# MCV-Univalle/HM-OpenCL

Measured on AMD Instinct MI355X. Metric: GSAD/s, higher is better.
Workload: dtype u8

## Files before the change

### hm-opencl_amd/csrc/hmme.hip

```cpp
#include "../../include/hmme.h"
#include "../../include/hmme_test.h"

#include <hip/hip_runtime.h>

#include <climits>
#include <cmath>
#include <cstdarg>
#include <cstdio>
#include <cstdlib>
#include <cstring>
#include <functional>
#include <string>
#include <type_traits>
#include <vector>

#include "me_kernels.hpp"

using hmme::MeJob;
using hmme::MeJob16;
using hmme::RefSet;

namespace {
constexpr int kMarginX = 128;
constexpr int kMarginY = 80;
// ... 1194 lines not shown
    if (t < best * 0.999) { best = t; best_k = k; }
  }
  return best_k;
}

static int plan_tail8(int tail, int slots, int w, int tail_knob) {
  if (tail <= 0 || tail >= hmme::kSegPrepThreads) return 0;
  const int nt = hmme::me_num_tasks(w, w), units = (nt + hmme::kSegUnit - 1) / hmme::kSegUnit;
  const long total = (long)tail * units;
  int best_wgs = 0;
  double best = (double)units + 0.25;
  for (int rounds = 1; rounds <= 4; ++rounds) {
    const long wgs = std::max<long>(1, std::min<long>((long)rounds * slots, total));
    const double per_wg = (double)total / wgs;
    const double t = 1.08 * rounds * (std::ceil(per_wg) + 0.25 * (1.0 + (per_wg - 1.0) / units)) + 0.5;
    if (t < best * 0.999) { best = t; best_wgs = (int)wgs; }
    if (wgs < (long)rounds * slots) break;
  }
  if (tail_knob > 1) best_wgs = (int)std::max<long>(1, std::min<long>((long)tail * tail_knob, total));
  return best_wgs;
}
static bool tail_one_launch(int head, int n_tail, int launches_knob) { return launches_knob == 1 || (launches_knob != 2 && 3 * n_tail >= head); }

static FramePlan plan_search(int jobs, int n_refs, int slots, int search_range, bool wide, const Knobs& knobs) {
  FramePlan pl;
  const int w = 2 * search_range + 1, tail = jobs % slots;
  pl.jobs = pl.tail_first = jobs;
  if (wide) {
    pl.mode = SearchMode::kStrips16;
    pl.pdw = pick_pdw16(w);
    const int rmax = pl.strip_rows = rows_max16(pl.pdw), n_min = strips_for(pl.pdw, w);
    const int h = hmme::me_strip_rows16(w, w, rmax, n_min + 4);
    pl.n_strips = (w + h - 1) / h;
    const int lanes = (((w + 1) >> 1) + 2) / 3;
    auto strip_cost = [&](int k) {
      const int hk = (w + k - 1) / k;
      return 2.0 * ((((hk * lanes + 63) >> 6) + 3) >> 2) + 1.0;
    };
    if (tail && knobs.tail_parts != 1) {
      const int k_max = std::min(w / 4, 64);
      int k = knobs.tail_parts > 1 ? std::min(knobs.tail_parts, k_max) : plan_tail(tail, slots, pl.n_strips, k_max, strip_cost);
      if (k < pl.n_strips) k = pl.n_strips;
      if (k > pl.n_strips) { pl.tail_first = jobs - tail; pl.tail_parts = k; }
    }
    pl.n_wg16 = pl.tail_first * pl.n_strips + (jobs - pl.tail_first) * pl.tail_parts;
    pl.table_bytes = sizeof(MeJob16) * (size_t)pl.n_wg16;
  } else if (search_range > 64) {
    pl.mode = SearchMode::kTiles8;
    pl.table_bytes = sizeof(MeJob16) * (size_t)jobs * 4;
  } else {
    const int wgs = tail && knobs.tail_parts != 1 ? plan_tail8(tail, slots, w, knobs.tail_parts) : 0;
    if (wgs > 0) { pl.tail_first = jobs - tail; pl.tail_wgs = wgs; }
    const int head = pl.tail_first, n_tail = jobs - head;
    if (!n_tail) {
      pl.table_bytes = sizeof(MeJob) * (size_t)head;
    } else if (tail_one_launch(head, n_tail, knobs.tail_launches)) {
      pl.mode = SearchMode::kSegments8;
      pl.table_bytes = hmme::me_seg_table_bytes(head + wgs, jobs);
    } else {
      pl.mode = SearchMode::kHeadThenSegments8;
      pl.tail_jobs_off = (sizeof(MeJob) * (size_t)head + 255) & ~(size_t)255;
      pl.table_bytes = pl.tail_jobs_off + hmme::me_seg_table_bytes(wgs, n_tail);
    }
  }
  pl.first_strip = pl.mode != SearchMode::kWhole8;
  const size_t per_ref = n_refs > 0 ? (pl.table_bytes + n_refs - 1) / n_refs : pl.table_bytes;
  pl.table_grow = per_ref * hmme::kMaxRefs + 4096;
  return pl;
}
static FramePlan plan_launch(const hmme_ctx* ctx, const hmme_frame_params* fp, int count, int n_refs, bool force16 = false) {
  return plan_search(count * n_refs, n_refs, ctx->wg_slots, fp->search_range, fp->bit_depth > 8 || force16, knobs());
}

int hmme_test_tail_plan(int width, int height, int search_range, int n_pairs, int slots, int* out) {
  if (!out || width < 8 || height < 8 || width > 16384 || height > 16384 || search_range < 1 || search_range > 64 || n_pairs < 1 || slots < 1) return HMME_ERR_ARG;
  const FramePlan pl = plan_search(hmme_num_ctus(width, height) * n_pairs, n_pairs, slots, search_range, false, Knobs{});
  out[0] = pl.jobs; out[1] = pl.tail_first; out[2] = pl.tail_wgs; out[3] = pl.mode == SearchMode::kSegments8 ? 1 : 0;
  return HMME_OK;
}

int hmme_test_pk_gate(uint32_t lambda_q16) { return hmme::me_pk_gate(lambda_q16) ? 1 : 0; }
int hmme_test_pk_body(uint32_t lambda_q16, int fen) { return hmme::me_pk_body(lambda_q16, fen ? 1 : 0); }
int hmme_test_pk_task_marker_free(int wx, int wy, int k, int it0, int n_it) { return hmme::me_task_marker_free(wx, wy, k, it0, n_it) ? 1 : 0; }

static int prep_jobs(hmme_ctx* ctx, const hmme_plane* cur, const hmme_frame_params* fp, const void* d_pred_q, int first, int count,
                     int n_refs, hipStream_t s, const FramePlan& pl, const void* d_center_q = nullptr) {
  const int jobs = pl.jobs, head = pl.tail_first, n_tail = jobs - head, w = cur->width, h = cur->height, sr = fp->search_range;
  bool moved;
  int rc = ensure(ctx, ctx->buf[kJobs], pl.table_bytes, pl.table_grow, &moved);
  if (moved) ctx->jobs_tag.valid = false;
  if (rc) return rc;
  if (pl.first_strip) {
    rc = ensure(ctx, ctx->buf[kFirstStrip], sizeof(int) * (size_t)jobs, sizeof(int) * (size_t)(jobs / (n_refs > 0 ? n_refs : 1) + 1) * hmme::kMaxRefs, &moved);
    if (moved) ctx->jobs_tag.valid = false;
    if (rc) return rc;
  }
  void* const d_jobs = ctx->buf[kJobs].p;
  int* const d_first_strip = ctx->buf[kFirstStrip].as<int>();
  hmme_ctx::TableTag tag;
  tag.valid = !d_pred_q && !d_center_q;
  tag.w = w; tag.h = h; tag.sr = sr; tag.first = first; tag.count = count; tag.pairs = n_refs;
  tag.bit_depth = fp->bit_depth | (pl.mode == SearchMode::kStrips16 && fp->bit_depth == 8 ? 0x100 : 0);
  tag.buf = d_jobs; tag.buf2 = pl.first_strip ? d_first_strip : nullptr; tag.stream = (void*)s;
  if (tag.same(ctx->jobs_tag)) return HMME_OK;
  ctx->jobs_tag.valid = false;
  const dim3 block(256);
  const auto grid = [](int n) { return dim3((n + 255) / 256); };
  const int16_t* pred = (const int16_t*)d_pred_q;
  switch (pl.mode) {
    case SearchMode::kTiles8:
      hipLaunchKernelGGL(hmme::me_prep_jobs_tile_kernel, grid(jobs), block, 0, s, (MeJob16*)d_jobs, d_first_strip, pred, first, count, n_refs, w, h, sr);
      break;
    case SearchMode::kStrips16:
      hipLaunchKernelGGL(hmme::me_prep_jobs16_kernel, grid(jobs), block, 0, s, (MeJob16*)d_jobs, d_first_strip, pred, first, count, n_refs, w, h, sr,
                         pl.n_strips, pl.strip_rows, pl.tail_first, pl.tail_parts, (const int16_t*)d_center_q);
      break;
    case SearchMode::kWhole8:
    case SearchMode::kSegments8:
    case SearchMode::kHeadThenSegments8: {
      const int idx0 = pl.mode == SearchMode::kSegments8 ? head : 0;
      if (head && idx0)
        hipLaunchKernelGGL(hmme::me_prep_whole_segments_kernel, grid(head), block, 0, s, d_jobs, d_first_strip, pred, first, count, n_refs, w, h, sr,
                           head + pl.tail_wgs, head);
      else if (head)
        hipLaunchKernelGGL(hmme::me_prep_jobs_kernel, grid(head), block, 0, s, (MeJob*)d_jobs, pred, first, count, n_refs, w, h, sr, 0, head, 1,
                           (uint32_t*)nullptr, (const int16_t*)nullptr);
      if (n_tail)
        hipLaunchKernelGGL(hmme::me_prep_segments_kernel, dim3(1), dim3(hmme::kSegPrepThreads), 0, s, (void*)((uint8_t*)d_jobs + pl.tail_jobs_off), d_first_strip,
                           pred, first, count, n_refs, w, h, sr, idx0 + pl.tail_wgs, head, n_tail, idx0);
      break;
    }
  }
  HIP_TRY(ctx, hipGetLastError());
  ctx->jobs_tag = tag;
  return HMME_OK;
}

static int run_search(hmme_ctx* ctx, const RefSet& curs, int cur_ctus_x, const RefSet& refs, int ref_pitch, const hmme_frame_params* fp, const FramePlan& pl,
                      int16_t* d_mv, uint32_t* d_sad, hipStream_t s) {
  const int head = pl.tail_first, n_tail = pl.jobs - head;
  const bool one_launch = pl.mode == SearchMode::kSegments8;
  const void* const d_jobs = ctx->buf[kJobs].p;
  const int* const d_first_strip = ctx->buf[kFirstStrip].as<int>();
  switch (pl.mode) {
    case SearchMode::kStrips16:
      return launch_search16(ctx, curs, cur_ctus_x, refs, ref_pitch, (const MeJob16*)d_jobs, d_first_strip, pl.jobs, pl.n_wg16,
                             pl.pdw, pl.strip_rows, fp->fen, fp->bit_depth, d_mv, d_sad, s);
    case SearchMode::kTiles8:
      return launch_search8_split(ctx, curs, cur_ctus_x, refs, ref_pitch, (const MeJob16*)d_jobs, d_first_strip, pl.jobs, 4,
                                  fp->fen, d_mv, d_sad, s);
    case SearchMode::kWhole8:
      return launch_search8<0>(ctx, curs, cur_ctus_x, refs, ref_pitch, d_jobs, head, fp->fen, d_mv, d_sad, nullptr, 0, s);
    case SearchMode::kSegments8:
    case SearchMode::kHeadThenSegments8: break;
  }
  unsigned long long* best = nullptr;
  int rc = merge_table(ctx, one_launch ? pl.jobs : n_tail, nullptr, s, &best);
  if (rc) return rc;
  if (one_launch)
    return launch_search8_segments(ctx, curs, cur_ctus_x, refs, ref_pitch, d_jobs, d_first_strip, pl.jobs, head + pl.tail_wgs, fp->fen, d_mv, d_sad, s, best);
  rc = launch_search8<0>(ctx, curs, cur_ctus_x, refs, ref_pitch, d_jobs, head, fp->fen, d_mv, d_sad, nullptr, 0, s);
  if (rc) return rc;
  return launch_search8_segments(ctx, curs, cur_ctus_x, refs, ref_pitch, (const uint8_t*)d_jobs + pl.tail_jobs_off, d_first_strip, n_tail, pl.tail_wgs,
                                 fp->fen, d_mv + (size_t)head * 2 * HMME_NUM_CTU_PARTS, d_sad + (size_t)head * HMME_NUM_CTU_PARTS, s, best);
}

// ... 2426 lines not shown
```

### hm-opencl_amd/csrc/me_kernels.hpp

```cpp
#pragma once

#include <hip/hip_runtime.h>
#include <stdint.h>

namespace hmme {

constexpr int kParts = 593;
constexpr int kPDW = 49;
constexpr int kWinRowsMax = 192;
constexpr int kIdxBits = 10;
constexpr uint32_t kInvCost = 3146751u;
constexpr int kGroups = 10;
constexpr int kIterPerTask = 4;
constexpr int kIterPerTaskSplit = 1;
static_assert(kIterPerTask == 4 && kIterPerTaskSplit <= 4, "2 iteration bits in the key; the guided schedule deals 4 / 2 / 1");
constexpr int kThreads = 256;

struct MeJob {
  int16_t ctu_x, ctu_y;
  int16_t lt_x, lt_y;
  int16_t rb_x, rb_y;
  int16_t pred_x, pred_y;
};
static_assert(sizeof(MeJob) == 16, "MeJob layout");
constexpr int kMaxRefs = 16;
struct RefSet { const uint8_t* base[kMaxRefs]; };

#include "me_slotmap.inc"

typedef uint16_t u16x4_t __attribute__((ext_vector_type(4)));
typedef uint32_t u32x2_t __attribute__((ext_vector_type(2)));
typedef __attribute__((address_space(3))) char lds_char_t;
typedef volatile __attribute__((address_space(3))) uint64_t lds_vu64_t;
typedef volatile __attribute__((address_space(3), aligned(4))) uint64_t lds_vu64a4_t;

__device__ __forceinline__ uint64_t me_pkadd(uint64_t a, uint64_t b) { return a + b; }
__device__ __forceinline__ uint64_t me_pksub(uint64_t a, uint64_t b) {
  return ((uint64_t)((uint32_t)(a >> 32) - (uint32_t)(b >> 32)) << 32) | (uint64_t)((uint32_t)a - (uint32_t)b);
}

#define ME_MAXKEY 0xFFFFFFFFu
#define ME_QSAD(pair, cur, acc) __builtin_amdgcn_qsad_pk_u16_u8((pair), (cur), (acc))
#define ME_KEYS(v, p, mult)                                                                                    \
  uint32_t v##_0, v##_1, v##_2, v##_3;                                                                         \
  asm volatile("v_mad_u32_u16 %0, %1, %2, %3" : "=v"(v##_0) : "v"((uint32_t)(p)), "s"(mult), "v"(c0));                   \
  asm volatile("v_mad_u32_u16 %0, %1, %2, %3 op_sel:[1,0,0,0]" : "=v"(v##_1) : "v"((uint32_t)(p)), "s"(mult), "v"(c1));   \
  asm volatile("v_mad_u32_u16 %0, %1, %2, %3" : "=v"(v##_2) : "v"((uint32_t)((p) >> 32)), "s"(mult), "v"(c2));           \
  asm volatile("v_mad_u32_u16 %0, %1, %2, %3 op_sel:[1,0,0,0]" : "=v"(v##_3) : "v"((uint32_t)((p) >> 32)), "s"(mult), "v"(c3))
#define ME_LIN(v, a, b)                                                                                         \
  uint32_t v##_0, v##_1, v##_2, v##_3;                                                                          \
  asm volatile("v_add3_u32 %0, %1, %2, %3" : "=v"(v##_0) : "v"(a##_0), "v"(b##_0), "v"(nc0));                              \
  asm volatile("v_add3_u32 %0, %1, %2, %3" : "=v"(v##_1) : "v"(a##_1), "v"(b##_1), "v"(nc1));                              \
  asm volatile("v_add3_u32 %0, %1, %2, %3" : "=v"(v##_2) : "v"(a##_2), "v"(b##_2), "v"(nc2));                              \
  asm volatile("v_add3_u32 %0, %1, %2, %3" : "=v"(v##_3) : "v"(a##_3), "v"(b##_3), "v"(nc3))
#define ME_SUB(v, a, b)                                                                                         \
  uint32_t v##_0, v##_1, v##_2, v##_3;                                                                          \
  asm volatile("v_sad_u32 %0, %1, %2, %3" : "=v"(v##_0) : "v"(a##_0), "v"(b##_0), "v"(c0));                                \
  asm volatile("v_sad_u32 %0, %1, %2, %3" : "=v"(v##_1) : "v"(a##_1), "v"(b##_1), "v"(c1));                                \
  asm volatile("v_sad_u32 %0, %1, %2, %3" : "=v"(v##_2) : "v"(a##_2), "v"(b##_2), "v"(c2));                                \
  asm volatile("v_sad_u32 %0, %1, %2, %3" : "=v"(v##_3) : "v"(a##_3), "v"(b##_3), "v"(c3))
__device__ __forceinline__ uint32_t me_min4(uint32_t a, uint32_t b, uint32_t c, uint32_t d) {
  uint32_t r;
  asm volatile("v_min3_u32 %0, %1, %2, %3\n\tv_min_u32 %0, %0, %4" : "=&v"(r) : "v"(a), "v"(b), "v"(c), "v"(d));
  return r;
}
#define ME_MIN4(k) me_min4(k##_0, k##_1, k##_2, k##_3)
#define ME_SUBMIN4(r, a, b)                                                                                     \
  uint32_t r;                                                                                                   \
  {                                                                                                             \
    uint32_t r##_t, r##_u;                                                                                      \
    asm volatile("v_sad_u32 %0, %3, %7, %11\n\tv_sad_u32 %1, %4, %8, %12\n\tv_sad_u32 %2, %5, %9, %13\n\t"            \
                 "v_min3_u32 %0, %0, %1, %2\n\tv_sad_u32 %1, %6, %10, %14\n\tv_min_u32 %0, %0, %1"                    \
                 : "=&v"(r), "=&v"(r##_t), "=&v"(r##_u)                                                        \
                 : "v"(a##_0), "v"(a##_1), "v"(a##_2), "v"(a##_3), "v"(b##_0), "v"(b##_1), "v"(b##_2), "v"(b##_3), "v"(c0), "v"(c1),     \
                   "v"(c2), "v"(c3));                                                                           \
  }

constexpr uint32_t kPkSlotMax = 64 * 255;
constexpr uint32_t kPkMarker = 0xFFFFu - kPkSlotMax;
constexpr uint32_t kPkMaxBits = 2 * 37;
__host__ __device__ inline bool me_pk_gate(uint32_t lambda_q16) {
  const uint64_t prod = (uint64_t)lambda_q16 * kPkMaxBits;
  return prod <= 0xFFFFFFFFull && (prod >> 16) + kPkSlotMax < kPkMarker;
}
constexpr uint32_t kPk2SlotMax = 16 * 12 * 255;
__host__ __device__ inline bool me_pk2_gate(uint32_t lambda_q16) {
  const uint64_t prod = (uint64_t)lambda_q16 * kPkMaxBits;
  return prod <= 0xFFFFFFFFull && (prod >> 16) + kPk2SlotMax <= 0xFFFFu;
}
__host__ __device__ inline int me_pk_body(uint32_t lambda_q16, int fen) {
  return (fen && me_pk2_gate(lambda_q16)) ? 2 : me_pk_gate(lambda_q16) ? 1 : 0;
}
__host__ __device__ inline bool me_task_marker_free(int wx, int wy, int k, int it0, int n_it) {
  if (!(wx & 3)) return true;
  const int quads = (wx + 3) >> 2;
  if ((quads & -quads) == (1 << k)) return false;
  const bool fold = (quads & 32) && (quads & 31) && (wy & 1);
  return !(fold && k == 5 && 2 * (it0 + n_it) > wy);
}
#define ME_PKMIN(r, p) ME_PKMIN_Q(r, (p) + pkm)
#define ME_PKMINE(r, p) ME_PKMIN_Q(r, ((p) << 1) + pkm)
#define ME_PKMIN_Q(r, q)                                                                                        \
  uint32_t r;                                                                                                   \
  {                                                                                                             \
    const uint64_t r##_q = (q);                                                                                 \
    asm volatile("v_pk_min_u16 %0, %1, %2\n\tv_pk_min_u16 %0, %0, %0 op_sel:[0,1] op_sel_hi:[1,0]\n\t"                \
                 "v_mad_u32_u16 %0, %0, %3, %4"                                                                 \
                 : "=&v"(r) : "v"((uint32_t)r##_q), "v"((uint32_t)(r##_q >> 32)), "s"(mult_a), "v"(ctag));      \
  }

#define ME_MERGE_DPP_MASKED(NAME, PAD, CTRL, MASK0)                                                          \
  __device__ __forceinline__ uint32_t NAME(uint32_t a, uint32_t b) {                                         \
    uint32_t r;                                                                                              \
    asm volatile(PAD "v_min_u32_dpp %0, %2, %2 " CTRL " row_mask:0xf bank_mask:0xf\n\t"                     \
        "v_min_u32_dpp %0, %1, %1 " CTRL " row_mask:0xf bank_mask:" MASK0                                    \
        : "=&v"(r) : "v"(a), "v"(b));                                                                        \
    return r;                                                                                                \
  }
ME_MERGE_DPP_MASKED(me_merge0, "s_nop 1\n\t", "row_ror:8", "0x3")
ME_MERGE_DPP_MASKED(me_merge1, "s_nop 1\n\t", "row_half_mirror", "0x5")
ME_MERGE_DPP_MASKED(me_merge0_nn, "", "row_ror:8", "0x3")
ME_MERGE_DPP_MASKED(me_merge1_nn, "", "row_half_mirror", "0x5")
__device__ __forceinline__ uint32_t me_merge2(uint32_t a, uint32_t b) {
  u32x2_t r = __builtin_amdgcn_permlane32_swap(a, b, false, false);
  return min(r.x, r.y);
}
__device__ __forceinline__ uint32_t me_merge3(uint32_t a, uint32_t b) {
  u32x2_t r = __builtin_amdgcn_permlane16_swap(a, b, false, false);
  return min(r.x, r.y);
}
template <int DPP_CTRL>
__device__ __forceinline__ uint32_t me_merge_dpp(uint32_t a, uint32_t b, bool role) {
  const uint32_t keep = role ? b : a;
  const uint32_t give = role ? a : b;
  return min(keep, (uint32_t)__builtin_amdgcn_update_dpp(0, (int)give, DPP_CTRL, 0xf, 0xf, false));
}
#define me_merge4(a, b, role) me_merge_dpp<0x4E>(a, b, role)
#define me_merge5(a, b, role) me_merge_dpp<0xB1>(a, b, role)

__device__ __forceinline__ uint32_t me_component_bits(int v) {
  const uint32_t t = (v <= 0) ? ((uint32_t)(-v) << 1) + 1u : ((uint32_t)v << 1);
  return 2u * (31u - (uint32_t)__builtin_clz(t)) + 1u;
}
__device__ __forceinline__ uint32_t me_mv_cost(uint32_t lambda_q16, int x, int y, int pred_x, int pred_y) {
  return (lambda_q16 * (me_component_bits((x << 2) - pred_x) + me_component_bits((y << 2) - pred_y))) >> 16;
}

__device__ __forceinline__ bool me_pk_slot(int s, bool wide, int& x, int& y, int& w, int& h) {
  if (s < 128) { x = (s & 7) * 8; y = (s >> 4) * 8 + ((s >> 3) & 1) * 4; w = 8; h = 4; return true; }
  if (s < 256) { x = ((s >> 1) & 7) * 8 + (s & 1) * 4; y = ((s - 128) >> 4) * 8; w = 4; h = 8; return true; }
  if (s >= 384 && s < 448) { x = (s & 7) * 8; y = ((s - 384) >> 3) * 8; w = 8; h = 8; return true; }
  if (!wide) return false;
  if (s < 384) {
    const int kk = (s - 256) >> 4;
    x = (s & 3) * 16; y = ((s >> 2) & 3) * 16; w = 16; h = 16;
    if (kk < 4) { h = kk < 2 ? 4 : 12; if (kk & 1) y += 16 - h; }
    else { w = kk < 6 ? 4 : 12; if (kk & 1) x += 16 - w; }
    return true;
  }
  if (s < 480) { x = (s & 3) * 16; y = ((s - 448) >> 3) * 16 + ((s >> 2) & 1) * 8; w = 16; h = 8; return true; }
  if (s < 512) { x = ((s >> 1) & 3) * 16 + (s & 1) * 8; y = ((s - 480) >> 3) * 16; w = 8; h = 16; return true; }
  return false;
}
template <int RW, int NR, int STEP>
__device__ __forceinline__ void me_pk_sads(const uint32_t* wrow, int pdw, const uint8_t* __restrict__ crow, uint32_t sad[4]) {
  constexpr int ND = RW / 4;
  static_assert(RW * NR * 255 <= 0xFFFF, "the four sums are packed u16");
  typedef uint64_t __attribute__((aligned(4))) u64a4_t;
  uint32_t c[NR][ND];
  uint64_t d[NR][ND];
#pragma unroll
  for (int r = 0; r < NR; ++r) {
#pragma unroll
    for (int k = 0; k < ND; ++k) c[r][k] = *(const uint32_t*)(crow + r * STEP * 64 + 4 * k);
#pragma unroll
    for (int k = 0; k < ND; ++k) d[r][k] = *(const u64a4_t*)(wrow + r * STEP * pdw + k);
  }
  uint64_t acc = 0;
#pragma unroll
  for (int r = 0; r < NR; ++r)
#pragma unroll
    for (int k = 0; k < ND; ++k) acc = ME_QSAD(d[r][k], c[r][k], acc);
#pragma unroll
  for (int j = 0; j < 4; ++j) sad[j] = (uint32_t)(acc >> (16 * j)) & 0xFFFFu;
}
template <bool WIDE>
__device__ __forceinline__ unsigned long long me_pk_recover(unsigned long long v, int s, const uint32_t* win, int pdw, const uint8_t* __restrict__ cur_blk,
                                                            const MeJob& job, int wx, uint32_t lambda_q16) {
  int rx, ry, rw, rh;
  if (v == ~0ull || !me_pk_slot(s, WIDE, rx, ry, rw, rh)) return v;
  const int xq = (int)(v & 0xfffc), y = (int)((v >> 16) & 0xffff);
  const uint32_t cost = (uint32_t)(v >> 32);
  const uint32_t* wrow = win + (y + ry) * pdw + ((xq + rx) >> 2);
  const uint8_t* crow = cur_blk + ry * 64 + rx;
  uint32_t sad[4] = {0u, 0u, 0u, 0u};
  int sh = 0;
  if (!WIDE || max(rw, rh) <= 8) {
    if (rh == 4) me_pk_sads<8, 4, 1>(wrow, pdw, crow, sad);
    else if (rw == 4) me_pk_sads<4, 8, 1>(wrow, pdw, crow, sad);
    else me_pk_sads<8, 8, 1>(wrow, pdw, crow, sad);
  } else if (rh <= 8) {
    if (rh == 4) me_pk_sads<16, 4, 1>(wrow, pdw, crow, sad);
    else me_pk_sads<16, 8, 1>(wrow, pdw, crow, sad);
  } else {
    sh = 1;
    if (rh == 12) me_pk_sads<16, 6, 2>(wrow, pdw, crow, sad);
    else if (rw == 4) me_pk_sads<4, 8, 2>(wrow, pdw, crow, sad);
    else if (rw == 8) me_pk_sads<8, 8, 2>(wrow, pdw, crow, sad);
    else me_pk_sads<12, 8, 2>(wrow, pdw, crow, sad);
  }
  const uint32_t by = me_component_bits(((job.lt_y + y) << 2) - job.pred_y);
  v &= ~3ull;
#pragma unroll
  for (int j = 0; j < 4; ++j)
    if (xq + j < wx && (sad[j] << sh) + ((lambda_q16 * (me_component_bits(((job.lt_x + xq + j) << 2) - job.pred_x) + by)) >> 16) == cost) return v + (unsigned long long)j;
  return v;
}

constexpr int kIdxBits16 = 8;
constexpr uint32_t kInvCost16 = 8000000u;
constexpr int kThreads16 = 256;

struct MeJob16 {
  MeJob j;
  int16_t y0, y1;
  int32_t job;
};

__host__ __device__ inline int me_xcd_unit(int p, int n) {
  const int x = p & 7, base = n >> 3, rem = n & 7;
  return x * base + (x < rem ? x : rem) + (p >> 3);
}
__host__ __device__ inline int me_xcd_position(int q, int n) {
  const int base = n >> 3, rem = n & 7, big = rem * (base + 1);
  if (q < big) return (q % (base + 1)) * 8 + q / (base + 1);
  const int r = q - big;
  return (r % base) * 8 + rem + r / base;
}

__host__ __device__ inline bool me_fold(int quads, int wy) { return (quads & 32) && (quads & 31) && (wy & 1); }
__host__ __device__ inline int me_num_tasks(int wx, int wy, int iter_per_task = kIterPerTaskSplit) {
  const int quads = (wx + 3) >> 2;
  const int wy_low = me_fold(quads, wy) ? wy - 1 : wy;
  int n = 0;
  for (int k = 5; k >= 0; --k)
    if (quads & (1 << k)) n += (((k == 5 ? wy : wy_low) + (64 >> k) - 1) / (64 >> k) + iter_per_task - 1) / iter_per_task;
  return n;
}
static_assert(sizeof(MeJob16) == 24, "MeJob16 layout");

constexpr int kGuidedT4 = 8, kGuidedT2 = 2;
__host__ __device__ inline void me_guided(int iters, int& n4, int& n2, int& n1) {
  n4 = iters > kGuidedT4 ? (iters - kGuidedT4 + 3) >> 2 : 0;
  const int rem = iters - 4 * n4;
  n2 = rem > kGuidedT2 ? (rem - kGuidedT2 + 1) >> 1 : 0;
  n1 = rem - 2 * n2;
}
__host__ __device__ inline int me_num_tasks_guided(int wx, int wy) {
  const int quads = (wx + 3) >> 2;
  const int wy_low = me_fold(quads, wy) ? wy - 1 : wy;
  int n = 0;
  for (int k = 5; k >= 0; --k)
    if (quads & (1 << k)) {
      int n4, n2, n1;
      me_guided(((k == 5 ? wy : wy_low) + (64 >> k) - 1) / (64 >> k), n4, n2, n1);
      n += n4 + n2 + n1;
    }
  return n;
}

__host__ __device__ inline int me_strip_rows16(int wx, int wy, int rows_max, int max_strips) {
  const int lanes = (((wx + 1) >> 1) + 2) / 3;
  int best_h = (wy + max_strips - 1) / max_strips, best_cost = 0x7fffffff;
  for (int n = (wy + rows_max - 1) / rows_max; n <= max_strips && n <= wy; ++n) {
    const int h = (wy + n - 1) / n;
    const int used = (wy + h - 1) / h, rest = wy - (used - 1) * h;
    const int cost = 2 * ((used - 1) * ((((h * lanes + 63) >> 6) + 3) >> 2) + ((((rest * lanes + 63) >> 6) + 3) >> 2)) + used;
    if (cost < best_cost) { best_cost = cost; best_h = h; }
  }
  return best_h;
}

constexpr int kBlkBytes8 = 64 * 64, kBlkBytes16 = 2 * 64 * 64;
template <int LINES>
__device__ __forceinline__ void me_prefetch_cur(uint64_t curc) {
  uint32_t d = 0;
#pragma unroll
  for (int l = 0; l < 64 * LINES; ++l) asm volatile("s_load_dword %0, %1, %2" : "+s"(d) : "s"(curc), "n"(64 * l));
  asm volatile("s_waitcnt lgkmcnt(0)" : "+s"(d));
}

template <int PDW, int THREADS>
__device__ __forceinline__ void me_stage_window(uint32_t* win, const uint32_t* __restrict__ src_al, int pitch_dw, int n, uint32_t mis, int tid) {
  constexpr int U = 8;
  for (int i0 = tid; i0 < n; i0 += THREADS * U) {
    uint32_t lo[U], hi[U];
#pragma unroll
    for (int u = 0; u < U; ++u) {
      const int i = min(i0 + u * THREADS, n - 1);
// ... 89 lines not shown
  const int quads = (wx + 3) >> 2;
  constexpr int kIt = SPLIT ? kIterPerTaskSplit : kIterPerTask;
  constexpr bool kGuided = !SPLIT;
  const int n_tasks = kGuided ? me_num_tasks_guided(wx, wy) : min(me_num_tasks(wx, wy, kIt), t_end);
  const bool fold = me_fold(quads, wy);
  const int wy_low = fold ? wy - 1 : wy;

  const uint32_t mult_a = 1u << kIdxBits;
  const uint32_t mult_e = FEN ? (2u << kIdxBits) : (1u << kIdxBits);
  const bool rb1 = lane & 2, rb0 = lane & 1;
  int prio_quarter = 0x0fffffff;
  if (fair_prio) {
    if constexpr (!SPLIT) {
      int total = 0;
      for (int kk = 5; kk >= 0; --kk)
        if (quads & (1 << kk)) total += ((kk == 5 ? wy : wy_low) + (64 >> kk) - 1) / (64 >> kk);
      prio_quarter = max(1, (total + 15) >> 4);
    } else {
      prio_quarter = max(1, ((n_tasks - t_first) * kIt + 15) >> 4);
    }
  }
  int prio_state = prio_quarter << 2;

  static_assert(SPLIT != 2 || kIterPerTaskSplit == 1, "segment mode counts tasks in lane-iterations");
  int grab_next = 0, grab_end = 0;
  while (true) {
    int t = 0;
    if constexpr (SPLIT == 2) {
      if (grab_next >= grab_end) {
        int want = 0;
        if (lane == 0) {
          const int left = n_tasks - *(volatile int*)&task_ctr;
          want = min(4, max(1, (left + 3) >> 2));
          t = atomicAdd(&task_ctr, want);
        }
        t = __builtin_amdgcn_readfirstlane(t);
        want = __builtin_amdgcn_readfirstlane(want);
        if (t >= n_tasks) break;
        grab_next = t; grab_end = min(t + want, n_tasks);
      }
      t = grab_next;
    } else {
      if (lane == 0) t = atomicAdd(&task_ctr, 1);
      t = __builtin_amdgcn_readfirstlane(t);
      if (t >= n_tasks) break;
    }
    if (prio_state < 4 && (prio_state & 3) < 3) {
      prio_state += (prio_quarter << 2) + 1;
      if ((prio_state & 3) == 1) __builtin_amdgcn_s_setprio(2);
      else if ((prio_state & 3) == 2) __builtin_amdgcn_s_setprio(1);
      else __builtin_amdgcn_s_setprio(0);
    }
    int x0 = 0, k = 0, it0 = 0, n_it = 0;
    {
      int xq = 0, rem = t;
      for (int kk = 5; kk >= 0; --kk) {
        if (!(quads & (1 << kk))) continue;
        const int iters = ((kk == 5 ? wy : wy_low) + (64 >> kk) - 1) / (64 >> kk);
        int nt;
        if constexpr (kGuided) {
          int n4, n2, n1;
          me_guided(iters, n4, n2, n1);
          nt = n4 + n2 + n1;
          if (rem < nt) {
            x0 = xq * 4; k = kk;
            if (rem < n4) { it0 = 4 * rem; n_it = 4; }
            else if (rem < n4 + n2) { it0 = 4 * n4 + 2 * (rem - n4); n_it = 2; }
            else { it0 = 4 * n4 + 2 * n2 + (rem - n4 - n2); n_it = 1; }
            break;
          }
        } else {
          nt = (iters + kIt - 1) / kIt;
          if (rem < nt) {
            x0 = xq * 4; k = kk; it0 = rem * kIt; n_it = min(kIt, iters - it0);
            if constexpr (SPLIT == 2) { n_it = min(grab_end - grab_next, iters - it0); grab_next += n_it; }
            break;
          }
        }
        rem -= nt;
        xq += 1 << kk;
      }
    }
    const int ty = 64 >> k;
    const int lx = lane & ((1 << k) - 1), ly = lane >> k;
    const bool fold_part = fold && k == 5;
    const bool marker_free = PK == 2 && me_task_marker_free(wx, wy, k, it0, n_it);

    uint32_t b0 = ME_MAXKEY, b1 = ME_MAXKEY, b2 = ME_MAXKEY, b3 = ME_MAXKEY, b4 = ME_MAXKEY, b5 = ME_MAXKEY,
             b6 = ME_MAXKEY, b7 = ME_MAXKEY, b8 = ME_MAXKEY, b9 = ME_MAXKEY;

    prio_state -= n_it << 2;
    for (int it = 0; it < n_it; ++it) {
      int cx = x0 + 4 * lx, cy = (it0 + it) * ty + ly;
      if (fold_part && cy == wy) { cx += 128; cy = wy - 1; }
      const bool vy = cy < wy;
      const int mvy = job.lt_y + cy, mvx = job.lt_x + cx;
      const uint32_t by = me_component_bits((mvy << 2) - job.pred_y);
      uint32_t lane_now = (uint32_t)lane;
      asm("" : "+v"(lane_now));
      const uint32_t tag = ((uint32_t)it << 8) | (lane_now << 2);
      uint32_t cc[4];
#pragma unroll
      for (int j = 0; j < 4; ++j) {
        const uint32_t cost = (lambda_q16 * (me_component_bits(((mvx + j) << 2) - job.pred_x) + by)) >> 16;
        cc[j] = (((vy && (cx + j) < wx) ? cost : kInvCost) << kIdxBits) | tag | (uint32_t)j;
      }
      const uint32_t c0 = cc[0], c1 = cc[1], c2 = cc[2], c3 = cc[3];
      const uint32_t nc0 = 0u - c0, nc1 = 0u - c1, nc2 = 0u - c2, nc3 = 0u - c3;
      uint64_t pkm = 0;
      uint32_t ctag = 0;
      if constexpr (PK) {
        const uint32_t m0 = cc[0] < (kInvCost << kIdxBits) ? cc[0] >> kIdxBits : kPkMarker, m1 = cc[1] < (kInvCost << kIdxBits) ? cc[1] >> kIdxBits : kPkMarker;
        const uint32_t m2 = cc[2] < (kInvCost << kIdxBits) ? cc[2] >> kIdxBits : kPkMarker, m3 = cc[3] < (kInvCost << kIdxBits) ? cc[3] >> kIdxBits : kPkMarker;
        pkm = (uint64_t)(m0 | m1 << 16) | (uint64_t)(m2 | m3 << 16) << 32;
        ctag = ((vy && cx < wx) ? 0u : kInvCost << kIdxBits) | tag;
      }
      const lds_char_t* lpc = (const lds_char_t*)(win + min(cy, wy - 1) * kPDW + (min(cx, wx - 1) >> 2));
#define ME8_CUR(row, q)                                                                                                            \
  ({                                                                                                                               \
    uint64_t w_;                                                                                                                   \
    asm volatile("s_load_dwordx2 %0, %1, %2" : "=s"(w_) : "s"(curc), "n"((row) * 64 + 8 * (q)));                                    \
    w_;                                                                                                                            \
  })
#define ME8_CUR_WAIT(w0, w1, w2, w3, w4, w5, w6, w7, d0, d1, d2, d3, d4, d5, d6, d7, d8, d9, d10, d11, d12, d13, d14, d15)           \
  asm volatile("" : : "v"(d0), "v"(d1), "v"(d2), "v"(d3), "v"(d4), "v"(d5), "v"(d6), "v"(d7), "v"(d8), "v"(d9), "v"(d10), "v"(d11),  \
               "v"(d12), "v"(d13), "v"(d14), "v"(d15));                                                                             \
  asm volatile("s_waitcnt lgkmcnt(0)" : "+s"(w0), "+s"(w1), "+s"(w2), "+s"(w3), "+s"(w4), "+s"(w5), "+s"(w6), "+s"(w7))
      if constexpr (PK == 2) {
        static_assert(PK != 2 || FEN == 1, "the marker-free body exists for FEN 1");
        if (marker_free) {
#include "me_tree_pk2_fen1.inc"
        } else {
#include "me_tree_pk_fen1.inc"
        }
      } else if constexpr (PK) {
        if constexpr (FEN) {
#include "me_tree_pk_fen1.inc"
        } else {
#include "me_tree_pk_fen0.inc"
        }
      } else if constexpr (FEN) {
#include "me_tree_fen1.inc"
      } else {
#include "me_tree_fen0.inc"
      }
    }

#define ME_FLUSH(g, key_)                                                                                          \
    {                                                                                                              \
      const int slot = ME_SLOT_OF[g][lane];                                                                        \
      const uint32_t key = (key_);                                                                                 \
      const uint32_t cost = key >> kIdxBits;                                                                       \
      if (slot >= 0 && cost < kInvCost) {                                                                          \
        const int kit = (key >> 8) & 3, kl = (key >> 2) & 63, kj = key & 3;                                        \
        int bx = x0 + 4 * (kl & ((1 << k) - 1)) + kj;                                                              \
        int byy = (it0 + kit) * ty + (kl >> k);                                                                    \
        if (fold_part && byy == wy) { bx += 128; byy = wy - 1; }                                                   \
        atomicMin(&best64[slot],                                                                                   \
                  ((unsigned long long)cost << 32) | ((unsigned long long)byy << 16) | (unsigned long long)bx);    \
      }                                                                                                            \
    }
    ME_FLUSH(0, b0) ME_FLUSH(1, b1) ME_FLUSH(2, b2) ME_FLUSH(3, b3) ME_FLUSH(4, b4)
    ME_FLUSH(5, b5) ME_FLUSH(6, b6) ME_FLUSH(7, b7) ME_FLUSH(8, b8) ME_FLUSH(9, b9)
#undef ME_FLUSH
  }
#ifdef ME_SEARCH_T_TIMELINE
  const unsigned long long tl_dry = wall_clock64();
#endif
  __syncthreads();
#ifdef ME_SEARCH_T_TIMELINE
  const unsigned long long tl_all = wall_clock64();
#endif

  if constexpr (SPLIT) {
    for (int s = tid; s < kParts; s += kThreads) {
      unsigned long long v = best64[s];
      if constexpr (PK) v = me_pk_recover<PK == 2>(v, s, win, kPDW, (const uint8_t*)cur_addr, job, wx, lambda_q16);
      if (v != ~0ull) atomicMin(&g_best[(long)out_job * kParts + s], v + tile_off);
    }
    if constexpr (SPLIT == 2) {
      if (seg_g < seg_end) continue;
    }
    return;
  }
  for (int s = tid; s < kParts; s += kThreads) {
    unsigned long long v = best64[s];
    if constexpr (PK) v = me_pk_recover<PK == 2>(v, s, win, kPDW, (const uint8_t*)cur_addr, job, wx, lambda_q16);
    const int mvx = job.lt_x + (int)(v & 0xffff), mvy = job.lt_y + (int)((v >> 16) & 0xffff);
    const uint32_t cost = (uint32_t)(v >> 32);
    const long o = (long)out_job * kParts + s;
    out_mv[2 * o] = (int16_t)mvx;
    out_mv[2 * o + 1] = (int16_t)mvy;
    out_sad[o] = cost - me_mv_cost(lambda_q16, mvx, mvy, job.pred_x, job.pred_y);
  }
#ifdef ME_SEARCH_T_TIMELINE
  __syncthreads();
  if (lane == 0) {
    uint32_t* o = out_sad + (long)out_job * kParts;
    const int wv = tid >> 6;
    if (wv == 0) {
      const unsigned long long t1 = wall_clock64();
      uint32_t hw_id;
      asm volatile("s_getreg_b32 %0, hwreg(HW_REG_HW_ID)" : "=s"(hw_id));
      uint32_t xcc_id;
      asm volatile("s_getreg_b32 %0, hwreg(HW_REG_XCC_ID)" : "=s"(xcc_id));
      o[0] = (uint32_t)tl_start; o[1] = (uint32_t)(tl_start >> 32); o[2] = (uint32_t)(tl_staged - tl_start); o[3] = (uint32_t)(tl_all - tl_start);
      o[4] = (uint32_t)(t1 - tl_start); o[5] = hw_id; o[6] = xcc_id; o[7] = blockIdx.x;
    }
    o[8 + wv] = (uint32_t)(tl_dry - tl_start);
  }
#endif
  break;
  }
}


__host__ __device__ inline void clip_mv_q(int& x, int& y, int cu_x, int cu_y, int pic_w, int pic_h) {
  const int hor_max = (pic_w + 8 - cu_x - 1) << 2, hor_min = (-64 - 8 - cu_x + 1) << 2;
  const int ver_max = (pic_h + 8 - cu_y - 1) << 2, ver_min = (-64 - 8 - cu_y + 1) << 2;
  x = (int16_t)(x > hor_max ? hor_max : (x < hor_min ? hor_min : x));
  y = (int16_t)(y > ver_max ? ver_max : (y < ver_min ? ver_min : y));
}
__host__ __device__ inline void set_search_range(int pred_x, int pred_y, int sr, int cu_x, int cu_y, int pic_w,
                                                 int pic_h, int& lt_x, int& lt_y, int& rb_x, int& rb_y) {
  int px = pred_x, py = pred_y;
  clip_mv_q(px, py, cu_x, cu_y, pic_w, pic_h);
  int ltx = (int16_t)(px - (sr << 2)), lty = (int16_t)(py - (sr << 2));
  int rbx = (int16_t)(px + (sr << 2)), rby = (int16_t)(py + (sr << 2));
  clip_mv_q(ltx, lty, cu_x, cu_y, pic_w, pic_h);
  clip_mv_q(rbx, rby, cu_x, cu_y, pic_w, pic_h);
  lt_x = ltx >> 2; lt_y = lty >> 2; rb_x = rbx >> 2; rb_y = rby >> 2;
}

// ... 2408 lines not shown
```

### hm-opencl_amd/hmme/api.py

```python
import ctypes as C
import os
import subprocess

import numpy as np

HERE = os.path.dirname(os.path.abspath(__file__))
CSRC = os.path.join(os.path.dirname(HERE), "csrc")
LIB_PATH = os.environ.get("HMME_LIB", os.path.join(CSRC, "libhmme.so"))
NUM_PARTS = 593

SYMBOLS = ["hmme_create", "hmme_destroy", "hmme_last_error", "hmme_device_info", "hmme_set_lambda",
           "hmme_set_lambda_q16", "hmme_get_lambda_q16", "hmme_params_ocl_compat", "hmme_set_search_range",
           "hmme_slot_index", "hmme_slot_rect", "hmme_slot_index_amp_off", "hmme_amp_off_slot", "hmme_compact_amp_off", "hmme_search_ctu", "hmme_search_ctu_w", "hmme_search_refine_ctu_w", "hmme_refine_ctu_w", "hmme_search_refine_ctu", "hmme_refine_ctu", "hmme_plane_create", "hmme_plane_create_ex", "hmme_plane_bit_depth", "hmme_plane_destroy", "hmme_plane_upload_pel",
           "hmme_plane_upload_u8", "hmme_host_register", "hmme_host_unregister", "hmme_plane_set_device_u8", "hmme_plane_width", "hmme_plane_height",
           "hmme_num_ctus", "hmme_search_frame", "hmme_search_frame_device", "hmme_search_frame_multi",
           "hmme_search_frame_multi_device", "hmme_refine_frame", "hmme_refine_frame_multi_device",
           "hmme_search_pairs_device", "hmme_refine_pairs_device", "hmme_plane_upload_async",
           "hmme_upload_status", "hmme_abi_version", "hmme_build_id", "hmme_device_index", "hmme_set_error_printing",
           "hmme_weight_check", "hmme_search_pairs_w_device", "hmme_refine_pairs_w_device", "hmme_search_frame_w", "hmme_refine_frame_w",
           "hmme_bipred_check", "hmme_predict_pairs_device", "hmme_predict_frame", "hmme_search_pairs_bi_device", "hmme_refine_pairs_bi_device",
           "hmme_search_frame_bi", "hmme_refine_frame_bi",
           "hmme_bipred_weight_check", "hmme_predict_pairs_w_device", "hmme_predict_frame_w", "hmme_search_pairs_bi_w_device",
           "hmme_refine_pairs_bi_w_device", "hmme_search_frame_bi_w", "hmme_refine_frame_bi_w",
           "hmme_slot_key", "hmme_select_check", "hmme_select_pairs_device", "hmme_select_frame",
           "hmme_ref_idx_bits", "hmme_select_refs_check", "hmme_select_refs_device", "hmme_select_refs_frame",
           "hmme_predict_refs_device", "hmme_predict_refs_frame",
           "hmme_select_dirs_check", "hmme_select_dirs_device", "hmme_select_dirs_frame", "hmme_predict_bi_device", "hmme_predict_bi_frame",
           "hmme_predict_bi_weight_check", "hmme_predict_bi_w_device", "hmme_predict_bi_w_frame", "hmme_predict_refs_w_device", "hmme_predict_refs_w_frame",
           "hmme_plane_stats", "hmme_wp_estimate", "hmme_wp_estimate_420",
           "hmme_predict_chroma_pairs_device", "hmme_predict_chroma_frame", "hmme_predict_chroma_refs_device", "hmme_predict_chroma_refs_frame",
           "hmme_predict_refs4_device", "hmme_predict_refs4_frame", "hmme_predict_chroma_refs4_device", "hmme_predict_chroma_refs4_frame",
           "hmme_predict_chroma_bi_device", "hmme_predict_chroma_bi_frame",
           "hmme_residual_pairs_device", "hmme_residual_frame",
           "hmme_search_frame_bi_refs_device", "hmme_refine_frame_bi_refs_device", "hmme_search_frame_bi_refs", "hmme_refine_frame_bi_refs",
           "hmme_select_dirs_refs_check", "hmme_select_dirs_refs_device", "hmme_select_dirs_refs_frame",
           "hmme_predict_bi_refs_device", "hmme_predict_bi_refs_frame",
           "hmme_bipred_refs_weight_check", "hmme_search_frame_bi_refs_w_device", "hmme_refine_frame_bi_refs_w_device", "hmme_search_frame_bi_refs_w",
           "hmme_refine_frame_bi_refs_w",
           "hmme_predict_bi_refs_weight_check", "hmme_predict_bi_refs_w_device", "hmme_predict_bi_refs_w_frame",
           "hmme_predict_chroma_bi_refs_device", "hmme_predict_chroma_bi_refs_frame"]
TEST_SYMBOLS = ["hmme_test_time_search_kernel", "hmme_test_device_address", "hmme_test_frac_deal", "hmme_test_tail_plan", "hmme_test_stage_layout", "hmme_test_picture_job", "hmme_test_time_weight_passes", "hmme_test_time_bipred_origin",
                "hmme_test_time_wp_estimate_passes", "hmme_test_pk_gate", "hmme_test_pk_body", "hmme_test_pk_task_marker_free",
                "hmme_test_wp_parameters", "hmme_test_wp_select", "hmme_test_ctu_plan"]
ABI_VERSION = 6


class HmmeError(RuntimeError):
    pass


class SearchParams(C.Structure):
    _fields_ = [("lt_x", C.c_int), ("lt_y", C.c_int), ("rb_x", C.c_int), ("rb_y", C.c_int),
                ("pred_x", C.c_int), ("pred_y", C.c_int), ("fen", C.c_int), ("bit_depth", C.c_int),
                ("shift_free", C.c_int)]


class Weight(C.Structure):
    _fields_ = [("w0", C.c_int), ("offset", C.c_int), ("shift", C.c_int), ("round", C.c_int)]


class WpInfo(C.Structure):
    _fields_ = [("cur_dc_sum", C.c_int64), ("cur_ac", C.c_int64), ("ref_dc_sum", C.c_int64), ("ref_ac", C.c_int64),
                ("sad_wp", C.c_int64), ("sad_nowp", C.c_int64),
                ("log2_denom", C.c_int), ("weight", C.c_int), ("offset", C.c_int), ("present", C.c_int),
                ("served_search", C.c_int), ("served_refine", C.c_int)]

    def as_dict(self):
        return {k: int(getattr(self, k)) for k, _ in self._fields_}


class SelectParams(C.Structure):
    _fields_ = [("mv_per_ctu", C.c_int), ("mv_unit", C.c_int), ("price_mv", C.c_int), ("part_mask", C.c_uint),
                ("min_depth", C.c_int), ("max_depth", C.c_int), ("cu_cost", C.c_uint32), ("pu_cost", C.c_uint32)]

    def __init__(self, mv_per_ctu=64, mv_unit=0, price_mv=0, part_mask=0xF7, min_depth=0, max_depth=3, cu_cost=0, pu_cost=0):
        super().__init__(int(mv_per_ctu), int(mv_unit), int(price_mv), int(part_mask), int(min_depth), int(max_depth), int(cu_cost), int(pu_cost))


class DirParams(C.Structure):
    _fields_ = [("dir_bits", C.c_uint32 * 3), ("list_bits", C.c_uint32 * 2)]

    def __init__(self, dir_bits=(0, 0, 0), list_bits=(0, 0)):
        super().__init__((C.c_uint32 * 3)(*[int(v) for v in dir_bits]), (C.c_uint32 * 2)(*[int(v) for v in list_bits]))


class DirRefsParams(C.Structure):
    _fields_ = [("dir_bits", C.c_uint32 * 3), ("n_refs", C.c_int * 2), ("ref_bits", (C.c_uint32 * 8) * 2), ("l1_valid_mask", C.c_uint32)]

    def __init__(self, dir_bits=(0, 0, 0), n_refs=(1, 1), ref_bits=((), ()), l1_valid_mask=None):
        rb = ((C.c_uint32 * 8) * 2)()
        for l in range(2):
            for r, v in enumerate(ref_bits[l]):
                rb[l][r] = int(v)
        mask = (1 << int(n_refs[1])) - 1 if l1_valid_mask is None else int(l1_valid_mask)
        super().__init__((C.c_uint32 * 3)(*[int(v) for v in dir_bits]), (C.c_int * 2)(*[int(v) for v in n_refs]), rb, mask)


class FrameParams(C.Structure):
    _fields_ = [("search_range", C.c_int), ("fen", C.c_int), ("bit_depth", C.c_int),
                ("ctu_first", C.c_int), ("ctu_count", C.c_int)]


def build():
    subprocess.run(["make", "-s", "-C", CSRC], check=True)


_lib = None


def load():
    global _lib
    if _lib is not None:
        return _lib
    if not os.path.exists(LIB_PATH):
        raise HmmeError(f"{LIB_PATH} is missing: build it with `make -C {CSRC}` (python __graft_entry__.py). "
                        "The engine has no CPU fallback.")
    L = C.CDLL(LIB_PATH)
    vp, i = C.c_void_p, C.c_int
    if not hasattr(L, "hmme_abi_version") or L.hmme_abi_version() != ABI_VERSION:
        raise HmmeError(f"{LIB_PATH}: ABI version {L.hmme_abi_version() if hasattr(L, 'hmme_abi_version') else '< 3'}, "
                        f"these bindings need {ABI_VERSION}: rebuild with `make -C {CSRC}`")
    L.hmme_build_id.restype = C.c_char_p
    L.hmme_create.argtypes = [i, i, C.c_uint, C.POINTER(vp)]
    L.hmme_destroy.argtypes = [vp]
    L.hmme_destroy.restype = None
# ... 1061 lines not shown
```

Before: 3799.

## Add full-task PK path with lane remapping and permlane-swap min merges

Replaces the marker-free packed-SAD body with a 'full task' body for tasks whose candidates are all valid. It remaps lanes so the partition-tree merges can use v_permlane32/16_swap plus packed u16 min in place of DPP keyed merges, and it uses a new slot map to match. It also changes the post-search pixel recovery so wide partitions scan up to 16 columns instead of 4, which lets the packed min lose the x index bits. This adds a new include file and test hook, and it depends on the remapped lanes and the slot map staying consistent.

```diff
diff --git a/hm-opencl_amd/csrc/hmme.hip b/hm-opencl_amd/csrc/hmme.hip
--- a/hm-opencl_amd/csrc/hmme.hip
+++ b/hm-opencl_amd/csrc/hmme.hip
@@ -1300,6 +1300,7 @@
 int hmme_test_pk_gate(uint32_t lambda_q16) { return hmme::me_pk_gate(lambda_q16) ? 1 : 0; }
 int hmme_test_pk_body(uint32_t lambda_q16, int fen) { return hmme::me_pk_body(lambda_q16, fen ? 1 : 0); }
 int hmme_test_pk_task_marker_free(int wx, int wy, int k, int it0, int n_it) { return hmme::me_task_marker_free(wx, wy, k, it0, n_it) ? 1 : 0; }
+int hmme_test_pk_task_full(int wx, int wy, int k, int it0, int n_it) { return hmme::me_task_full(wx, wy, k, it0, n_it) ? 1 : 0; }
 
 static int prep_jobs(hmme_ctx* ctx, const hmme_plane* cur, const hmme_frame_params* fp, const void* d_pred_q, int first, int count,
                      int n_refs, hipStream_t s, const FramePlan& pl, const void* d_center_q = nullptr) {
diff --git a/hm-opencl_amd/csrc/me_kernels.hpp b/hm-opencl_amd/csrc/me_kernels.hpp
--- a/hm-opencl_amd/csrc/me_kernels.hpp
+++ b/hm-opencl_amd/csrc/me_kernels.hpp
@@ -27,6 +27,7 @@
 struct RefSet { const uint8_t* base[kMaxRefs]; };
 
 #include "me_slotmap.inc"
+#include "me_slotmap3.inc"
 
 typedef uint16_t u16x4_t __attribute__((ext_vector_type(4)));
 typedef uint32_t u32x2_t __attribute__((ext_vector_type(2)));
@@ -98,6 +99,13 @@
   const bool fold = (quads & 32) && (quads & 31) && (wy & 1);
   return !(fold && k == 5 && 2 * (it0 + n_it) > wy);
 }
+__host__ __device__ inline bool me_task_full(int wx, int wy, int k, int it0, int n_it) {
+  if (k < 2) return false;
+  const int quads = (wx + 3) >> 2;
+  if ((wx & 3) && (quads & -quads) == (1 << k)) return false;
+  const bool fold = (quads & 32) && (quads & 31) && (wy & 1);
+  return (it0 + n_it) * (64 >> k) <= ((k == 5 || !fold) ? wy : wy - 1);
+}
 #define ME_PKMIN(r, p) ME_PKMIN_Q(r, (p) + pkm)
 #define ME_PKMINE(r, p) ME_PKMIN_Q(r, ((p) << 1) + pkm)
 #define ME_PKMIN_Q(r, q)                                                                                        \
@@ -108,6 +116,34 @@
                  "v_mad_u32_u16 %0, %0, %3, %4"                                                                 \
                  : "=&v"(r) : "v"((uint32_t)r##_q), "v"((uint32_t)(r##_q >> 32)), "s"(mult_a), "v"(ctag));      \
   }
+
+#define ME_PKMIN16_LO(r, q)                                                                                     \
+  uint32_t r;                                                                                                   \
+  {                                                                                                             \
+    const uint64_t r##_q = (q);                                                                                 \
+    asm volatile("v_pk_min_u16 %0, %1, %2\n\t"                                                                  \
+                 "v_min_u16_sdwa %0, %0, %0 dst_sel:WORD_0 dst_unused:UNUSED_PAD src0_sel:WORD_0 src1_sel:WORD_1" \
+                 : "=&v"(r) : "v"((uint32_t)r##_q), "v"((uint32_t)(r##_q >> 32)));                              \
+  }
+#define ME_PKMIN16_HI(r, q)                                                                                     \
+  {                                                                                                             \
+    const uint64_t r##_q = (q);                                                                                 \
+    uint32_t r##_t;                                                                                             \
+    asm volatile("v_pk_min_u16 %1, %2, %3\n\t"                                                                  \
+                 "v_min_u16_sdwa %0, %1, %1 dst_sel:WORD_1 dst_unused:UNUSED_PRESERVE src0_sel:WORD_0 src1_sel:WORD_1" \
+                 : "+v"(r), "=&v"(r##_t) : "v"((uint32_t)r##_q), "v"((uint32_t)(r##_q >> 32)));                 \
+  }
+#define ME_KEY16_LO(k, r) uint32_t k; asm volatile("v_mad_u32_u16 %0, %1, %2, %3" : "=v"(k) : "v"(r), "s"(mult_a), "v"(ctag))
+#define ME_KEY16_HI(k, r) uint32_t k; asm volatile("v_mad_u32_u16 %0, %1, %2, %3 op_sel:[1,0,0,0]" : "=v"(k) : "v"(r), "s"(mult_a), "v"(ctag))
+#define ME_PMERGE(NAME, PAD, SWAP)                                                                           \
+  __device__ __forceinline__ uint32_t NAME(uint32_t a, uint32_t b) {                                         \
+    asm volatile(PAD SWAP " %0, %1\n\tv_pk_min_u16 %0, %0, %1" : "+v"(a), "+v"(b));                          \
+    return a;                                                                                                \
+  }
+ME_PMERGE(me_pmerge2, "s_nop 1\n\t", "v_permlane32_swap_b32")
+ME_PMERGE(me_pmerge3, "s_nop 1\n\t", "v_permlane16_swap_b32")
+ME_PMERGE(me_pmerge2_nn, "", "v_permlane32_swap_b32")
+ME_PMERGE(me_pmerge3_nn, "", "v_permlane16_swap_b32")
 
 #define ME_MERGE_DPP_MASKED(NAME, PAD, CTRL, MASK0)                                                          \
   __device__ __forceinline__ uint32_t NAME(uint32_t a, uint32_t b) {                                         \
@@ -189,10 +225,15 @@
                                                             const MeJob& job, int wx, uint32_t lambda_q16) {
   int rx, ry, rw, rh;
   if (v == ~0ull || !me_pk_slot(s, WIDE, rx, ry, rw, rh)) return v;
-  const int xq = (int)(v & 0xfffc), y = (int)((v >> 16) & 0xffff);
+  const int x_first = (int)(v & 0xfffc), y = (int)((v >> 16) & 0xffff);
   const uint32_t cost = (uint32_t)(v >> 32);
+  const uint8_t* crow = cur_blk + ry * 64 + rx;
+  const uint32_t by = me_component_bits(((job.lt_y + y) << 2) - job.pred_y);
+  const int x_end = (WIDE && !(x_first & 12)) ? min(x_first + 16, wx) : x_first + 4;
+  v &= ~0xffffull;
+#pragma unroll 1
+  for (int xq = x_first; xq < x_end; xq += 4) {
   const uint32_t* wrow = win + (y + ry) * pdw + ((xq + rx) >> 2);
-  const uint8_t* crow = cur_blk + ry * 64 + rx;
   uint32_t sad[4] = {0u, 0u, 0u, 0u};
   int sh = 0;
   if (!WIDE || max(rw, rh) <= 8) {
@@ -209,12 +250,11 @@
     else if (rw == 8) me_pk_sads<8, 8, 2>(wrow, pdw, crow, sad);
     else me_pk_sads<12, 8, 2>(wrow, pdw, crow, sad);
   }
-  const uint32_t by = me_component_bits(((job.lt_y + y) << 2) - job.pred_y);
-  v &= ~3ull;
 #pragma unroll
   for (int j = 0; j < 4; ++j)
-    if (xq + j < wx && (sad[j] << sh) + ((lambda_q16 * (me_component_bits(((job.lt_x + xq + j) << 2) - job.pred_x) + by)) >> 16) == cost) return v + (unsigned long long)j;
-  return v;
+    if (xq + j < wx && (sad[j] << sh) + ((lambda_q16 * (me_component_bits(((job.lt_x + xq + j) << 2) - job.pred_x) + by)) >> 16) == cost) return v | (unsigned long long)(xq + j);
+  }
+  return v | (unsigned long long)x_first;
 }
 
 constexpr int kIdxBits16 = 8;
@@ -470,9 +510,10 @@
       }
     }
     const int ty = 64 >> k;
-    const int lx = lane & ((1 << k) - 1), ly = lane >> k;
+    const bool full = PK == 2 && me_task_full(wx, wy, k, it0, n_it);
+    int lx = lane & ((1 << k) - 1), ly = lane >> k;
+    if (full) { lx = ((lane >> 5) & 1) | ((lane >> 3) & 2) | ((lane & ((1 << (k - 2)) - 1)) << 2); ly = (lane & 15) >> (k - 2); }
     const bool fold_part = fold && k == 5;
-    const bool marker_free = PK == 2 && me_task_marker_free(wx, wy, k, it0, n_it);
 
     uint32_t b0 = ME_MAXKEY, b1 = ME_MAXKEY, b2 = ME_MAXKEY, b3 = ME_MAXKEY, b4 = ME_MAXKEY, b5 = ME_MAXKEY,
              b6 = ME_MAXKEY, b7 = ME_MAXKEY, b8 = ME_MAXKEY, b9 = ME_MAXKEY;
@@ -484,7 +525,7 @@
       const bool vy = cy < wy;
       const int mvy = job.lt_y + cy, mvx = job.lt_x + cx;
       const uint32_t by = me_component_bits((mvy << 2) - job.pred_y);
-      uint32_t lane_now = (uint32_t)lane;
+      uint32_t lane_now = (uint32_t)(ly << k | lx);
       asm("" : "+v"(lane_now));
       const uint32_t tag = ((uint32_t)it << 8) | (lane_now << 2);
       uint32_t cc[4];
@@ -502,6 +543,7 @@
         const uint32_t m2 = cc[2] < (kInvCost << kIdxBits) ? cc[2] >> kIdxBits : kPkMarker, m3 = cc[3] < (kInvCost << kIdxBits) ? cc[3] >> kIdxBits : kPkMarker;
         pkm = (uint64_t)(m0 | m1 << 16) | (uint64_t)(m2 | m3 << 16) << 32;
         ctag = ((vy && cx < wx) ? 0u : kInvCost << kIdxBits) | tag;
+        if (full) ctag = tag & ~(3u << 2);
       }
       const lds_char_t* lpc = (const lds_char_t*)(win + min(cy, wy - 1) * kPDW + (min(cx, wx - 1) >> 2));
 #define ME8_CUR(row, q)                                                                                                            \
@@ -515,9 +557,9 @@
                "v"(d12), "v"(d13), "v"(d14), "v"(d15));                                                                             \
   asm volatile("s_waitcnt lgkmcnt(0)" : "+s"(w0), "+s"(w1), "+s"(w2), "+s"(w3), "+s"(w4), "+s"(w5), "+s"(w6), "+s"(w7))
       if constexpr (PK == 2) {
-        static_assert(PK != 2 || FEN == 1, "the marker-free body exists for FEN 1");
-        if (marker_free) {
-#include "me_tree_pk2_fen1.inc"
+        static_assert(PK != 2 || FEN == 1, "the full-task body exists for FEN 1");
+        if (full) {
+#include "me_tree_pk3_fen1.inc"
         } else {
 #include "me_tree_pk_fen1.inc"
         }
@@ -536,7 +578,7 @@
 
 #define ME_FLUSH(g, key_)                                                                                          \
     {                                                                                                              \
-      const int slot = ME_SLOT_OF[g][lane];                                                                        \
+      const int slot = full ? ME_SLOT_OF3[g][lane] : ME_SLOT_OF[g][lane];                                          \
       const uint32_t key = (key_);                                                                                 \
       const uint32_t cost = key >> kIdxBits;                                                                       \
       if (slot >= 0 && cost < kInvCost) {                                                                          \
diff --git a/hm-opencl_amd/csrc/me_slotmap3.inc b/hm-opencl_amd/csrc/me_slotmap3.inc
--- /dev/null
+++ b/hm-opencl_amd/csrc/me_slotmap3.inc
@@ -0,0 +1,12 @@
+static __device__ const short ME_SLOT_OF3[10][64] = {
+  {0, 2, 25, 27, 131, 135, 480, 482, 8, 10, 146, 150, 385, 387, 481, 483, 384, 386, 448, 449, 144, 148, 320, 321, 1, 3, 452, 453, 145, 149, 336, 337, 128, 132, 147, 151, 16, 18, 288, 289, 129, 133, 393, 395, 24, 26, 304, 305, 9, 11, 256, 257, 392, 394, 352, 353, 130, 134, 272, 273, 17, 19, 368, 369},
+  {32, 34, 57, 59, 163, 167, 488, 490, 40, 42, 178, 182, 401, 403, 489, 491, 400, 402, 456, 457, 176, 180, 324, 325, 33, 35, 460, 461, 177, 181, 340, 341, 160, 164, 179, 183, 48, 50, 292, 293, 161, 165, 409, 411, 56, 58, 308, 309, 41, 43, 260, 261, 408, 410, 356, 357, 162, 166, 276, 277, 49, 51, 372, 373},
+  {4, 6, 29, 31, 139, 143, 484, 486, 12, 14, 154, 158, 389, 391, 485, 487, 388, 390, 450, 451, 152, 156, 322, 323, 5, 7, 454, 455, 153, 157, 338, 339, 136, 140, 155, 159, 20, 22, 290, 291, 137, 141, 397, 399, 28, 30, 306, 307, 13, 15, 258, 259, 396, 398, 354, 355, 138, 142, 274, 275, 21, 23, 370, 371},
+  {36, 38, 61, 63, 171, 175, 492, 494, 44, 46, 186, 190, 405, 407, 493, 495, 404, 406, 458, 459, 184, 188, 326, 327, 37, 39, 462, 463, 185, 189, 342, 343, 168, 172, 187, 191, 52, 54, 294, 295, 169, 173, 413, 415, 60, 62, 310, 311, 45, 47, 262, 263, 412, 414, 358, 359, 170, 174, 278, 279, 53, 55, 374, 375},
+  {64, 66, 89, 91, 195, 199, 496, 498, 72, 74, 210, 214, 417, 419, 497, 499, 416, 418, 464, 465, 208, 212, 328, 329, 65, 67, 468, 469, 209, 213, 344, 345, 192, 196, 211, 215, 80, 82, 296, 297, 193, 197, 425, 427, 88, 90, 312, 313, 73, 75, 264, 265, 424, 426, 360, 361, 194, 198, 280, 281, 81, 83, 376, 377},
+  {96, 98, 121, 123, 227, 231, 504, 506, 104, 106, 242, 246, 433, 435, 505, 507, 432, 434, 472, 473, 240, 244, 332, 333, 97, 99, 476, 477, 241, 245, 348, 349, 224, 228, 243, 247, 112, 114, 300, 301, 225, 229, 441, 443, 120, 122, 316, 317, 105, 107, 268, 269, 440, 442, 364, 365, 226, 230, 284, 285, 113, 115, 380, 381},
+  {68, 70, 93, 95, 203, 207, 500, 502, 76, 78, 218, 222, 421, 423, 501, 503, 420, 422, 466, 467, 216, 220, 330, 331, 69, 71, 470, 471, 217, 221, 346, 347, 200, 204, 219, 223, 84, 86, 298, 299, 201, 205, 429, 431, 92, 94, 314, 315, 77, 79, 266, 267, 428, 430, 362, 363, 202, 206, 282, 283, 85, 87, 378, 379},
+  {100, 102, 125, 127, 235, 239, 508, 510, 108, 110, 250, 254, 437, 439, 509, 511, 436, 438, 474, 475, 248, 252, 334, 335, 101, 103, 478, 479, 249, 253, 350, 351, 232, 236, 251, 255, 116, 118, 302, 303, 233, 237, 445, 447, 124, 126, 318, 319, 109, 111, 270, 271, 444, 446, 366, 367, 234, 238, 286, 287, 117, 119, 382, 383},
+  {544, 537, 540, 534, 548, 552, 547, 542, 545, 541, 546, 538, 549, 553, 550, 554, 584, 572, 571, 567, 516, 586, 513, 575, 512, 573, 585, 574, 520, 514, 517, 587, 560, 556, 551, 555, 568, 564, 563, 559, 562, 557, 561, 558, 569, 566, 570, 565, 524, 518, 521, 515, 532, 526, 529, 523, 528, 522, 525, 519, 536, 530, 533, 527},
+  {531, -1, 583, -1, 539, -1, -1, -1, 535, -1, -1, -1, 543, -1, -1, -1, 592, -1, -1, -1, 577, -1, -1, -1, 576, -1, -1, -1, 578, -1, -1, -1, 588, -1, -1, -1, 590, -1, -1, -1, 589, -1, -1, -1, 591, -1, -1, -1, 579, -1, -1, -1, 581, -1, -1, -1, 580, -1, -1, -1, 582, -1, -1, -1},
+};
diff --git a/hm-opencl_amd/hmme/api.py b/hm-opencl_amd/hmme/api.py
--- a/hm-opencl_amd/hmme/api.py
+++ b/hm-opencl_amd/hmme/api.py
@@ -40,7 +40,7 @@
            "hmme_predict_bi_refs_weight_check", "hmme_predict_bi_refs_w_device", "hmme_predict_bi_refs_w_frame",
            "hmme_predict_chroma_bi_refs_device", "hmme_predict_chroma_bi_refs_frame"]
 TEST_SYMBOLS = ["hmme_test_time_search_kernel", "hmme_test_device_address", "hmme_test_frac_deal", "hmme_test_tail_plan", "hmme_test_stage_layout", "hmme_test_picture_job", "hmme_test_time_weight_passes", "hmme_test_time_bipred_origin",
-                "hmme_test_time_wp_estimate_passes", "hmme_test_pk_gate", "hmme_test_pk_body", "hmme_test_pk_task_marker_free",
+                "hmme_test_time_wp_estimate_passes", "hmme_test_pk_gate", "hmme_test_pk_body", "hmme_test_pk_task_marker_free", "hmme_test_pk_task_full",
                 "hmme_test_wp_parameters", "hmme_test_wp_select", "hmme_test_ctu_plan"]
 ABI_VERSION = 6
 
```

Measured after the change: 4060 (median of 6 runs). +6.9%, better.
